# NYXFLOWER/TIP

Hardware: AMD Instinct MI355X
Metric: D-D edges aggregated/sec (encoder fwd+bwd) (higher is better)
Workload: dtype f32

## Files before the change

### include/tipk.h

```cpp
#ifndef TIPK_H
#define TIPK_H

#include <stdint.h>

#ifdef __cplusplus
extern "C" {
#endif

#define TIPK_ABI_VERSION 24

#define TIPK_OK            0
#define TIPK_EINVAL      (-1)
#define TIPK_EUNSUPPORTED (-2)
#define TIPK_EHIP_BASE   (-1000)

typedef void* tipk_stream_t;

int         tipk_abi_version(void);
const char* tipk_strerror(int status);
const char* tipk_build_id(void);
int         tipk_set_option(const char* name, int value);
int         tipk_get_option(const char* name, int* value);
int         tipk_device_info(int device, int* n_cu, int* lds_bytes_per_cu, int* wavefront, char* arch, int arch_len);

int tipk_gather_sum(const float* table, int64_t ld_table, int64_t n_table ,
                    const int32_t* row_id, const float* edge_w ,
                    const int32_t* items, int64_t n_items,
                    float* out, int64_t ld_out,
                    float* partial ,
                    const float* row_scale ,
                    const float* bias , int relu,
                    int d, int group_slots , tipk_stream_t stream);
// ... 122 lines not shown

int tipk_rgcn_dest_products_supported(int64_t n_nodes, int64_t n_rel, int n_bases, int d_in);
int tipk_rgcn_dest_products(const float* x, int64_t ld_x, int d_in, const float* att, int64_t ld_att, int n_bases,
                            int64_t n_nodes, int64_t n_rel, const int32_t* node_desc, const uint32_t* edges,
                            float* t, int64_t t_sb, int64_t t_sv, tipk_stream_t stream);

int tipk_sum_slabs_xb(const float* slabs, int64_t n_slabs, int64_t slab_stride, int64_t n_rows, int d_in,
                      const float* row_scale , const float* addend , int relu, float* x,
                      const float* basis, const float* root, int n_bases, int d_out, float* xb, float* xroot,
                      tipk_stream_t stream);

int tipk_rgcn_row_products_supported(int64_t n_nodes, int64_t n_rel, int n_bases, int channels);
int64_t tipk_rgcn_row_products_slabs(int64_t n_nodes, int channels);
int tipk_rgcn_row_products(const float* table, int64_t ld_table, int64_t n_nodes, int channels, const float* att,
                           int64_t ld_att, int64_t n_rel, int n_bases, const int32_t* entries, const int32_t* desc,
                           const float* xb , int64_t ld_xb, float* t, float* datt_slabs ,
                           tipk_stream_t stream);

int tipk_rgcn_row_products_s_supported(int64_t n_nodes, int64_t n_rel, int n_bases, int channels);
int tipk_rgcn_row_products_s(const float* table, int64_t ld_table, int64_t n_nodes, int channels, const float* att,
                             int64_t ld_att, int64_t n_rel, int n_bases, const int32_t* entries, const int32_t* desc,
                             const float* xb , int64_t ld_xb, float* t, float* datt_slabs ,
                             tipk_stream_t stream);

int tipk_transpose(const float* in, int64_t rows, int64_t cols, float* out, tipk_stream_t stream);

int tipk_rows_affine(const float* in, int64_t ld_in,
                     const float* row_mul, const float* row_div,
                     const float* gate, int64_t ld_gate,
                     float* out, int64_t ld_out,
                     int64_t rows, int64_t cols, int accumulate, tipk_stream_t stream);

int tipk_gate_colsum_groups(int64_t rows, int64_t cols);
int tipk_gate_colsum(const float* in, int64_t ld_in, const float* gate, int64_t ld_gate,
                     float* out, int64_t ld_out, int64_t rows, int64_t cols, float* scratch,
                     tipk_stream_t stream);

int tipk_drug_mix_fwd(const float* xd, int64_t ld_xd, const float* d_norm, const float* mean, int64_t ld_mean,
                      const float* w, int p, int q, int64_t rows, int ne, int cat, float* out, int64_t ld_out,
                      tipk_stream_t stream);

int tipk_drug_mix_gather_supported(int p, int q);
int tipk_drug_mix_gather_fwd(const float* xd, int64_t ld_xd, const float* d_norm, const float* h, int64_t ld_h,
                             const int32_t* ptr, const int32_t* src, const float* scale, const int32_t* wg_desc,
                             const int32_t* order , int64_t n_wg,
                             const float* w, int p, int q, int64_t rows, int ne, int cat, float* out, int64_t ld_out,
// ... 197 lines not shown
```

### tip_amd/_lib.py

```python
import ctypes as C
import glob
import hashlib
import os
import subprocess

import torch

_HERE = os.path.dirname(os.path.abspath(__file__))
LIB_PATH = os.path.join(_HERE, 'libtipk.so')
CSRC = os.path.join(_HERE, 'csrc')

ABI_VERSION = 24


class TipkError(RuntimeError):
    pass


class GemmDesc(C.Structure):
    _fields_ = [('m', C.c_int64), ('n', C.c_int64), ('k', C.c_int64),
                ('batch', C.c_int64), ('kbatch', C.c_int64), ('ksplit', C.c_int64),
                ('a', C.c_void_p), ('a_sm', C.c_int64), ('a_sk', C.c_int64), ('a_sq', C.c_int64), ('a_sz', C.c_int64),
                ('b', C.c_void_p), ('b_sk', C.c_int64), ('b_sn', C.c_int64), ('b_sq', C.c_int64), ('b_sz', C.c_int64),
                ('c', C.c_void_p), ('c_sm', C.c_int64), ('c_sz', C.c_int64), ('c_ss', C.c_int64),
                ('c_in', C.c_void_p), ('cin_sm', C.c_int64), ('cin_sz', C.c_int64),
                ('alpha', C.c_float), ('relu', C.c_int)]


class SlabSumDesc(C.Structure):
    _fields_ = [('in_', C.c_void_p), ('n_slabs', C.c_int64), ('slab_stride', C.c_int64), ('count', C.c_int64),
                ('alpha', C.c_float), ('accumulate', C.c_int),
                ('row_scale', C.c_void_p), ('cols', C.c_int64),
                ('addend', C.c_void_p), ('relu', C.c_int),
                ('gate', C.c_void_p),
                ('out', C.c_void_p)]
# ... 39 lines not shown
    'tipk_gather_sum': (_I, [_P, _L, _L, _P, _P, _P, _L, _P, _L, _P, _P, _P, _I, _I, _I, _P]),
    'tipk_gather_sum_finalize': (_I, [_P, _P, _L, _P, _L, _P, _P, _I, _I, _I, _P]),
    'tipk_gather_sum_riders_supported': (_I, [_I, _I]),
    'tipk_gather_sum_riders': (_I, [_P, _L, _L, _P, _P, _P, _L, _P, _L, _P, _P, _I, _I, _I, _P, _L, _P, C.POINTER(SlabSumDesc), C.c_int32, _P]),
    'tipk_gather_sum_lin_supported': (_I, [_I, _I, _I]),
    'tipk_gather_sum_lin': (_I, [_P, _L, _L, _P, _P, _P, _L, _P, _L, _P, _P, _L, _L, _P, _I, _P, _L, _I, _I, _I, _P]),
    'tipk_gather_rows_csr': (_I, [_P, _L, _L, _P, _P, _L, _P, _L, _I, _P]),
    'tipk_rel_gather_supported': (_I, [_L, _I, _I]),
    'tipk_rel_gather_occupancy': (_I, [_L, _I, _I]),
    'tipk_rel_gather_chunk': (_I, [_L, _I, _I]),
    'tipk_pair_product_supported': (_I, [_I, _I]),
    'tipk_pair_product': (_I, [_P, _P, _L, _L, _I, _I, _I, _I, _P, _P, _P, _P, _P]),
    'tipk_rgcn_pair_grads_supported': (_I, [_I, _I]),
    'tipk_rgcn_pair_grads': (_I, [_P, _L, _P, _P, _L, _L, _I, _I, _P, _P, _P, _L, _P, _L, _L, _P, _L, _P]),
    'tipk_stream_gather_parts': (_I, [_P, _L, _I, _L, _P, _L, _P, _L, _P, _P, _P, _I, _P, _P, _P, _L, _P]),
    'tipk_stream_gather_parts_two': (_I, [_P, _P, _L, _I, _L, _P, _L, _P, _L, _P, _P, _P, _I, _P, _P, _P, _P, _L, _P]),
    'tipk_rgcn_dest_products_supported': (_I, [_L, _L, _I, _I]),
    'tipk_rgcn_dest_products': (_I, [_P, _L, _I, _P, _L, _I, _L, _L, _P, _P, _P, _L, _L, _P]),
    'tipk_rgcn_row_products_supported': (_I, [_L, _L, _I, _I]),
    'tipk_rgcn_row_products_slabs': (_L, [_L, _I]),
    'tipk_rgcn_row_products': (_I, [_P, _L, _L, _I, _P, _L, _L, _I, _P, _P, _P, _L, _P, _P, _P]),
    'tipk_rgcn_row_products_s_supported': (_I, [_L, _L, _I, _I]),
    'tipk_rgcn_row_products_s': (_I, [_P, _L, _L, _I, _P, _L, _L, _I, _P, _P, _P, _L, _P, _P, _P]),
    'tipk_sum_slabs_xb': (_I, [_P, _L, _L, _L, _I, _P, _P, _I, _P, _P, _P, _I, _I, _P, _P, _P]),
    'tipk_stream_gather_supported': (_I, [_L, _I, _I]),
    'tipk_stream_gather_piece': (_I, []),
    'tipk_stream_gather_two': (_I, [_P, _P, _L, _L, _I, _L, _P, _P, _P, _I, _P, _P, _L, _P]),
    'tipk_stream_gather': (_I, [_P, _L, _L, _I, _L, _P, _P, _P, _I, _P, _P, _P, _P, _L, _I, _I, _P, _P, _I, _P]),
    'tipk_rel_gather': (_I, [_I, _P, _L, _L, _I, _L, _P, _P, _P, _I, _P, _P, _P, _P, _L, _P]),
    'tipk_gemm_f32': (_I, [C.POINTER(GemmDesc), _P]),
    'tipk_gemm_f32_group': (_I, [C.POINTER(GemmDesc), C.c_int32, _P]),
    'tipk_sum_slabs_group': (_I, [C.POINTER(SlabSumDesc), C.c_int32, _P]),
    'tipk_gemm_wg_group_supported': (_I, [C.POINTER(WgGemmDesc)]),
    'tipk_gemm_wg_group': (_I, [C.POINTER(WgGemmDesc), C.c_int32, C.POINTER(SlabSumDesc), C.c_int32, _P]),
    'tipk_rgcn_dy_products_plan': (_I, [_L, _L, _I, C.POINTER(_I), C.POINTER(_I)]),
    'tipk_rgcn_dy_products': (_I, [_P, _L, _P, _L, _P, _L, _L, _L, _I, _P, _L, _P, _P, _P]),
    'tipk_rgcn_node_products_plan': (_I, [_L, _I, _L, _I, C.POINTER(_I)]),
    'tipk_rgcn_node_products': (_I, [_P, _L, _I, _P, _P, _P, _L, _L, _P, _L, _I, _P, _L, _L, _P, _P, _L, _L, _P, _P]),
    'tipk_sum_slabs': (_I, [_P, _L, _L, _L, _F, _I, _P, _P]),
    'tipk_sum_slabs_ex': (_I, [_P, _L, _L, _L, _F, _I, _P, _L, _P, _I, _P, _P]),
    'tipk_transpose': (_I, [_P, _L, _L, _P, _P]),
    'tipk_rows_affine': (_I, [_P, _L, _P, _P, _P, _L, _P, _L, _L, _L, _I, _P]),
    'tipk_gate_colsum_groups': (_I, [_L, _L]),
    'tipk_gate_colsum': (_I, [_P, _L, _P, _L, _P, _L, _L, _L, _P, _P]),
    'tipk_drug_mix_fwd': (_I, [_P, _L, _P, _P, _L, _P, _I, _I, _L, _I, _I, _P, _L, _P]),
    'tipk_drug_mix_gather_supported': (_I, [_I, _I]),
# ... 177 lines not shown
```

### tip_amd/csrc/tipk_row_products.hip

```cpp
#include <stdlib.h>
#include <type_traits>
#include "tipk_common.h"

namespace {

typedef float f32x16 __attribute__((ext_vector_type(16)));
typedef unsigned int u32;
typedef __attribute__((address_space(3))) float rp_lds_f32_t;

constexpr int RP_WAVES = 8;
constexpr int RP_TLD = 33;

struct RpArgs {
    const float* table; u32 ld_table_b; int n_nodes, ch;
    const float* att; u32 ld_att_b; int R, NB;
    const float* xb; int64_t ld_xb;
    const int32_t* entries; const int32_t* desc; int n_tiles;
    float* t_out;
    float* datt;
    int n_groups;
    int dbg;
};

__device__ __forceinline__ float rp_ldg(const float* base, u32 byte_off) {
    return *reinterpret_cast<const float*>(reinterpret_cast<const char*>(base) + byte_off);
}
__device__ __forceinline__ float rp_and(float v, u32 mask) { return __uint_as_float(__float_as_uint(v) & mask); }
template <int I>
__device__ __forceinline__ u32 rp_row_bcast(u32 x) {
    return (u32)__builtin_amdgcn_update_dpp(0, (int)x, 0x150 + (I & 15), 0xf, 0xf, true);
}
template <int I>
__device__ __forceinline__ void rp_fmac_row_bcast(float& d, float x, float y) {
    asm("v_fmac_f32_dpp %0, %1, %2 row_newbcast:%3 row_mask:0xf bank_mask:0xf bound_ctrl:1" : "+v"(d) : "v"(x), "v"(y), "n"(I & 15));
}
__device__ __forceinline__ void rp_wave_sync() {
    __builtin_amdgcn_fence(__ATOMIC_RELEASE, "wavefront");
    __builtin_amdgcn_wave_barrier();
    __builtin_amdgcn_fence(__ATOMIC_ACQUIRE, "wavefront");
}
template <int N, int I = 0, typename F>
__device__ __forceinline__ void rp_static_for(F&& f) {
    if constexpr (I < N) {
// ... 191 lines not shown
                if constexpr ((g & 1) == 0) { consume(lo, va, wa); issue(lo_nx, va, g + 2 < NQ ? wa : wb); }
                else { consume(lo, vb, wa); issue(lo_nx, vb, g + 2 < NQ ? wa : wb); }
            });
            wa = wb; wb = wq[0];
#pragma unroll
            for (int q = 0; q + 1 < WQ; ++q) wq[q] = wq[q + 1];
            wq[WQ - 1] = load_word(b + 2 + WQ);
            ++b;
        } while (++i < nbat);
        finish_tile();
        nbat = nbat_next;
    }
    if (wave_on) {
#pragma unroll
        for (int q = 0; q < CPL; ++q)
#pragma unroll
            for (int r = 0; r < 16; ++r) {
                const int bb = (r & 3) + 8 * (r >> 2) + 4 * kh;
                if (bb < NB) a.t_out[(int64_t)bb * NC + col0 + 32 * q + row] = acc1[q][r];
            }
    }
}

constexpr int RPS_TS = 65;
constexpr int RPS_TILE = (33 * RPS_TS + 3) / 4 * 4;

template <bool P2>
__global__ __launch_bounds__(RP_WAVES * 64, 4) void row_products_s_kernel(RpArgs a) {
    constexpr int TS = RPS_TS;
    extern __shared__ __attribute__((aligned(16))) float lds[];
    const int t = threadIdx.x, lane = t & 63;
    const int w = __builtin_amdgcn_readfirstlane(t >> 6);
    const int row = lane & 31, kh = lane >> 5;
    float* tile = lds + w * RPS_TILE;
    float* attl = lds + RP_WAVES * RPS_TILE;
    const int cb = (int)blockIdx.x / a.n_groups, grp = (int)blockIdx.x - cb * a.n_groups;
    const int node_raw = grp * RP_WAVES + w;
    const bool wave_on = node_raw < a.n_nodes;
    const int node = wave_on ? node_raw : a.n_nodes - 1;
    const int NB = a.NB, R = a.R;
    const int64_t NC = (int64_t)a.n_nodes * a.ch;
    const int64_t col0 = (int64_t)node * a.ch + cb * 64;
    const u32 voff = (u32)(cb * 64 + lane) * 4u;
    u32 tile_base = __builtin_amdgcn_readfirstlane((u32)(uintptr_t)(rp_lds_f32_t*)tile);
    const u32 att_b = (u32)(row < NB ? row : NB - 1) * 4u;
    const __amdgpu_buffer_rsrc_t rsrc = __builtin_amdgcn_make_buffer_rsrc(const_cast<float*>(a.table), 0,
                                                                           (int)((u32)a.n_nodes * a.ld_table_b), 0x00020000);
    float xbv[2][16];
    if (P2) {
        const int64_t b_off = (int64_t)(row < NB ? row : NB - 1) * a.ld_xb + col0;
#pragma unroll
        for (int q = 0; q < 2; ++q)
#pragma unroll
            for (int kk = 0; kk < 16; ++kk)
                xbv[q][kk] = rp_and(a.xb[b_off + 32 * q + 2 * kk + kh], (row < NB && wave_on) ? 0xffffffffu : 0u);
    }
    f32x16 acc1[2];
#pragma unroll
    for (int q = 0; q < 2; ++q)
#pragma unroll
        for (int i = 0; i < 16; ++i) acc1[q][i] = 0.f;
    const int32_t* dsc = a.desc + (int64_t)node * a.n_tiles * 2;
    int b = __builtin_amdgcn_readfirstlane(dsc[0]);
    int nbat = __builtin_amdgcn_readfirstlane(dsc[1]);
    int tl = 0;
    float acc = 0.f;
    float atv[16];
    float va[8], vb[8];
    int w1c[16], wn[32];
    typedef const __attribute__((address_space(4))) int32_t* rp_const_i32_t;
    const rp_const_i32_t entries_c = (rp_const_i32_t)(uintptr_t)a.entries;
    auto load_words = [&](int batch, int (&dst)[32]) __attribute__((always_inline)) {
        const rp_const_i32_t eb = entries_c + (int64_t)batch * 32;
#pragma unroll
        for (int j = 0; j < 32; ++j) dst[j] = eb[j];
    };
    auto issue = [&](auto lo_c, float (&val)[8], const int (&w0)[32]) __attribute__((always_inline)) {
        constexpr int LO = decltype(lo_c)::value;
#pragma unroll
        for (int j = 0; j < 8; ++j)
            val[j] = __builtin_bit_cast(float, __builtin_amdgcn_raw_buffer_load_b32(rsrc, (int)voff, w0[LO + j], 0));
    };
    auto consume = [&](auto lo_c, float (&val)[8], const int (&w1)[16]) __attribute__((always_inline)) {
        constexpr int LO = decltype(lo_c)::value;
        const u32 tb = tile_base;
#pragma unroll
        for (int j = 0; j < 8; ++j) {
            const int wd = w1[LO + j];
            const float keep = __int_as_float(wd & 0x3f800000);
            acc = fmaf(acc, keep, val[j]);
            if (!TIPK_DBG(a.dbg & 2))
                asm volatile("s_add_u32 m0, %1, %2\n\ts_nop 0\n\tds_write_addtid_b32 %0" : : "v"(acc), "s"(tb), "s"(wd) : "memory", "scc");
        }
    };
    constexpr int NT = RP_WAVES * 64, PER = 1024 / NT;
    float att_next[PER];
    auto att_elem = [&](int tile_i, int i) __attribute__((always_inline)) {
        const int e = i * NT + t, r = tile_i * 32 + (e >> 5), bb = e & 31;
        const float v = a.att[(int64_t)(r < R ? r : R - 1) * (a.ld_att_b >> 2) + (bb < NB ? bb : NB - 1)];
        return rp_and(v, (r < R && bb < NB && tile_i < a.n_tiles) ? 0xffffffffu : 0u);
    };
    auto att_store = [&](int buf) __attribute__((always_inline)) {
#pragma unroll
        for (int i = 0; i < PER; ++i) attl[buf * (32 * RP_TLD) + ((i * NT + t) >> 5) * RP_TLD + (t & 31)] = att_next[i];
    };
    if (P2) {
#pragma unroll
        for (int i = 0; i < PER; ++i) att_next[i] = att_elem(0, i);
        att_store(0);
        __syncthreads();
    }
    auto begin_tile = [&]() __attribute__((always_inline)) {
        const int r0 = tl * 32;
        if (P2) {
#pragma unroll
            for (int i = 0; i < PER; ++i) att_next[i] = att_elem(tl + 1 < a.n_tiles ? tl + 1 : tl, i);
        } else {
            const float* att_t = a.att + (int64_t)r0 * (a.ld_att_b >> 2);
#pragma unroll
            for (int kk = 0; kk < 16; ++kk) {
                const int r = r0 + 2 * kk + kh;
                atv[kk] = rp_ldg(att_t, (u32)((r < R ? r : R - 1) - r0) * a.ld_att_b + att_b);
            }
            if (r0 + 32 > R || NB < 32) {
#pragma unroll
                for (int kk = 0; kk < 16; ++kk)
                    atv[kk] = rp_and(atv[kk], (r0 + 2 * kk + kh < R && row < NB) ? 0xffffffffu : 0u);
            }
        }
        constexpr int N4 = 32 * TS / 4;
        static_assert(32 * TS % 4 == 0, "tile zeroing");
#pragma unroll
        for (int i = 0; i < (N4 + 63) / 64; ++i)
            if (i * 64 + lane < N4) tipk_st4(tile + (i * 64 + lane) * 4, make_float4(0.f, 0.f, 0.f, 0.f));
        rp_wave_sync();
    };
    auto finish_tile = [&]() __attribute__((always_inline)) {
        const int r0 = tl * 32;
        rp_wave_sync();
        if (!TIPK_DBG(a.dbg & 4))
#pragma unroll
        for (int kk = 0; kk < 16; ++kk) {
            const float av = P2 ? attl[(tl & 1) * (32 * RP_TLD) + (2 * kk + kh) * RP_TLD + row] : atv[kk];
#pragma unroll
            for (int q = 0; q < 2; ++q)
                acc1[q] = __builtin_amdgcn_mfma_f32_32x32x2f32(av, tile[(2 * kk + kh) * TS + 32 * q + row], acc1[q], 0, 0, 0);
        }
        if (P2) {
            f32x16 acc2;
#pragma unroll
            for (int i = 0; i < 16; ++i) acc2[i] = 0.f;
#pragma unroll
            for (int q = 0; q < 2; ++q)
#pragma unroll
                for (int kk = 0; kk < 16; ++kk)
                    acc2 = __builtin_amdgcn_mfma_f32_32x32x2f32(tile[row * TS + 32 * q + 2 * kk + kh], xbv[q][kk], acc2, 0, 0, 0);
            att_store((tl + 1) & 1);
            rp_wave_sync();
#pragma unroll
            for (int r = 0; r < 16; ++r) {
                const int rr = (r & 3) + 8 * (r >> 2) + 4 * kh;
                tile[rr * 32 + row] = acc2[r];
            }
            __syncthreads();
#pragma unroll
            for (int i = 0; i < PER; ++i) {
                const int e = i * NT + t;
                float sum = lds[e];
#pragma unroll
                for (int q = 1; q < RP_WAVES; ++q) sum += lds[q * RPS_TILE + e];
                const int rr = r0 + (e >> 5), bb = e & 31;
                if (rr < R && bb < NB) a.datt[((int64_t)blockIdx.x * R + rr) * NB + bb] = sum;
            }
            __syncthreads();
        }
    };
    constexpr std::integral_constant<int, 0> c0{};
    constexpr std::integral_constant<int, 8> c8{};
    load_words(b, wn);
#pragma unroll
    for (int j = 0; j < 16; ++j) w1c[j] = wn[16 + j];
    issue(c0, va, wn);
    issue(c8, vb, wn);
    for (tl = 0; tl < a.n_tiles; ++tl) {
        const int nbat_next = __builtin_amdgcn_readfirstlane(dsc[2 * (tl + 1 < a.n_tiles ? tl + 1 : tl) + 1]);
        begin_tile();
        int i = 0;
        do {
            load_words(b + 1, wn);
            consume(c0, va, w1c);
            issue(c0, va, wn);
            consume(c8, vb, w1c);
            issue(c8, vb, wn);
#pragma unroll
            for (int j = 0; j < 16; ++j) w1c[j] = wn[16 + j];
            ++b;
        } while (++i < nbat);
        finish_tile();
        nbat = nbat_next;
    }
    if (wave_on) {
#pragma unroll
        for (int q = 0; q < 2; ++q)
#pragma unroll
            for (int r = 0; r < 16; ++r) {
                const int bb = (r & 3) + 8 * (r >> 2) + 4 * kh;
                if (bb < NB) a.t_out[(int64_t)bb * NC + col0 + 32 * q + row] = acc1[q][r];
            }
    }
}

template <bool P2>
int rps_launch(const RpArgs& a, unsigned blocks, hipStream_t st) {
    const size_t lds = (size_t)(RP_WAVES * RPS_TILE + (P2 ? 2 * 32 * RP_TLD : 0)) * sizeof(float);
    hipError_t e = hipFuncSetAttribute((const void*)row_products_s_kernel<P2>, hipFuncAttributeMaxDynamicSharedMemorySize, (int)lds);
    if (e != hipSuccess) return tipk_hip_status(e);
    hipLaunchKernelGGL((row_products_s_kernel<P2>), dim3(blocks), dim3(RP_WAVES * 64), lds, st, a);
    TIPK_RETURN_LAUNCH();
}

template <int CPL> constexpr size_t rp_lds_bytes(bool p2) {
    return (size_t)(RP_WAVES * RpGeom<CPL>::TILE + (p2 ? 2 * 32 * RP_TLD : 0)) * sizeof(float);
}

template <bool P2, int CPL>
int rp_launch(const RpArgs& a, unsigned blocks, hipStream_t st) {
    const size_t lds = rp_lds_bytes<CPL>(P2);
    hipError_t e = hipFuncSetAttribute((const void*)row_products_kernel<P2, CPL>, hipFuncAttributeMaxDynamicSharedMemorySize, (int)lds);
    if (e != hipSuccess) return tipk_hip_status(e);
    hipLaunchKernelGGL((row_products_kernel<P2, CPL>), dim3(blocks), dim3(RP_WAVES * 64), lds, st, a);
    TIPK_RETURN_LAUNCH();
}

inline int rp_cpl(int channels) { return channels % 64 == 0 ? 2 : 1; }

}

extern "C" int tipk_rgcn_row_products_supported(int64_t n_nodes, int64_t n_rel, int n_bases, int channels) {
    if (n_nodes <= 0 || n_rel <= 0 || n_bases <= 0 || n_bases > 32 || channels <= 0 || channels % 32 != 0) return 0;
    if (n_nodes > 65536 || n_rel > 0x7fffffffLL) return 0;
// ... 32 lines not shown

extern "C" int tipk_rgcn_row_products_s_supported(int64_t n_nodes, int64_t n_rel, int n_bases, int channels) {
    if (n_nodes <= 0 || n_rel <= 0 || n_bases <= 0 || n_bases > 32 || channels <= 0 || channels % 64 != 0) return 0;
    if (n_rel > 0x7fffffffLL || tipk_ceil_div(n_nodes, RP_WAVES) * (channels / 64) > 0x7fffffffLL) return 0;
    return 1;
}

extern "C" int tipk_rgcn_row_products_s(const float* table, int64_t ld_table, int64_t n_nodes, int channels, const float* att,
                                        int64_t ld_att, int64_t n_rel, int n_bases, const int32_t* entries, const int32_t* desc,
                                        const float* xb, int64_t ld_xb, float* t_out, float* datt_slabs, tipk_stream_t stream) {
    if (!tipk_rgcn_row_products_s_supported(n_nodes, n_rel, n_bases, channels)) return TIPK_EUNSUPPORTED;
    if (!table || !att || !entries || !desc || !t_out || ld_table < channels || ld_att < n_bases) return TIPK_EINVAL;
    if ((xb == nullptr) != (datt_slabs == nullptr) || (xb && ld_xb < n_nodes * channels)) return TIPK_EINVAL;
    if (n_nodes * ld_table * 4 >= (1LL << 31) || 32 * ld_att * 4 >= (1LL << 31)) return TIPK_EUNSUPPORTED;
    RpArgs a;
    a.table = table; a.ld_table_b = (u32)(ld_table * 4); a.n_nodes = (int)n_nodes; a.ch = channels;
    a.att = att; a.ld_att_b = (u32)(ld_att * 4); a.R = (int)n_rel; a.NB = n_bases;
    a.xb = xb; a.ld_xb = ld_xb;
    a.entries = entries; a.desc = desc; a.n_tiles = (int)tipk_ceil_div(n_rel, 32);
    a.t_out = t_out; a.datt = datt_slabs;
    a.n_groups = (int)tipk_ceil_div(n_nodes, RP_WAVES);
    a.dbg = TIPK_DBG(tipk_option(TIPK_OPT_DP_DEBUG));
    const unsigned blocks = (unsigned)(a.n_groups * (channels / 64));
    return xb ? rps_launch<true>(a, blocks, (hipStream_t)stream) : rps_launch<false>(a, blocks, (hipStream_t)stream);
}
```

### tip_amd/layers.py

```python
import math
import os
import pickle

import numpy as np
import torch
from torch import nn
from torch.nn import Parameter as Param

from . import encoder, ops, switches
from .data import Data, build_data_dict
from .neg_sampling import typed_negative_sampling
from .plan import (build_pair_bwd_plan, build_dest_plan, build_row_stream_plan, build_row_stream_plan_s, build_gather_plan, build_gather_plan_segmented, build_rel_plan, build_stream_plan, build_stream_plan_rows, build_csr_plan, group_slots_for,
                   relations_per_segment, DEFAULT_CHUNK)
from .utils import process_edges, auprc_auroc_ap_by_range

EPS = 1e-13

__all__ = ['GCNConv', 'MyRGCNConv', 'MyRGCNConv2', 'MyHierarchyConv', 'PPEncoder', 'FMEncoder',
           'FMEncoderCat', 'MultiInnerProductDecoder', 'NNDecoder', 'Setting', 'TIP']


def _ident(*tensors):
    key = []
    for t in tensors:
        if t is None:
            key.append(None)
        elif t.is_sparse:
            key.append((id(t), tuple(t.shape), str(t.device), t.dtype))
        else:
            key.append((t.data_ptr(), tuple(t.shape), t._version, str(t.device), t.dtype))
    return tuple(key)


class _PlanCache(object):

# ... 346 lines not shown
            pair_fwd = build_stream_plan_rows(src[keep] * n_nodes + dst[keep], rel[keep], n_nodes * n_nodes, n_rel, pair_wgs,
                                              (n_bases // split_p) // 4, ops.rel_stream_piece())
            pair_fwd.symmetric = symmetric
            pair_fwd.links = pair_link_words(src, dst, n_nodes)
        split_s = ops.rel_stream_split(n_nodes, d_out) if on_dev and n_rel * n_nodes < 2 ** 24 else 0
        if pair_fwd is not None and ops.pair_grads_supported(n_bases, d_out):
            sym, lanes_p = pair_fwd.symmetric, (n_bases // split_p) // 4
            pair_bwd = lambda: _shared_pair_bwd_plan(src, dst, rel, n_nodes, n_rel, 1.0 / deg, sym, pair_wgs, lanes_p, plan_share)
        if split_s:
            compact = bool(n_bases) and ops.node_products_slabs(n_nodes, d_out, n_rel, n_bases) > 0
            lanes_s = (d_out // split_s) // 4
            build_rs = lambda: build_stream_plan(src, dst, rel, n_nodes, n_rel, n_cu, lanes_s, ops.rel_stream_piece(), compact=compact)
            rs_bwd = build_rs if pair_bwd is not None else build_rs()
        else:
            rl_bwd = lambda: build_rel_plan(src, dst, rel, n_nodes, n_rel, wg_b, backward=True, lanes=lanes_b)
    dest_fwd = row_fwd = row_bwd = None
    wide = False
    if src.is_cuda and d_out and n_bases and pair_fwd is None and n_rel * n_nodes * d_out * 4 > (192 << 20):
        bits = ops.dest_products_bits(n_nodes, n_rel, n_bases, 1)
        if bits:
            dest_fwd = lambda: build_dest_plan(src, dst, rel, n_nodes, n_rel, bits)
        wide = bool(d_out) and d_out % 64 == 0 and ops.row_products_s_supported(n_nodes, n_rel, n_bases, d_out) \
            and n_nodes < (1 << 23) and n_nodes * d_out * 4 < 2 ** 31
        if wide:
            row_fwd = lambda: build_row_stream_plan_s(dst, src, rel, n_nodes, n_rel)
            row_bwd = lambda: build_row_stream_plan_s(src, dst, rel, n_nodes, n_rel)
        elif ops.row_products_supported(n_nodes, n_rel, n_bases, 32):
            row_fwd = lambda: build_row_stream_plan(dst, src, rel, n_nodes, n_rel)
            row_bwd = lambda: build_row_stream_plan(src, dst, rel, n_nodes, n_rel)

    def fwd_plan():
        y_bytes = n_rel * n_nodes * (d_out or 0) * 4
        ordered = rel.numel() < 2 or bool((rel[1:] >= rel[:-1]).all())
        if y_bytes > (192 << 20) and ordered:
            per = relations_per_segment(n_nodes, d_out)
            return build_gather_plan_segmented(dst, yrow, rel // per, n_nodes, n_rel * n_nodes, chunk, 'dd.fwd')
        return build_gather_plan(dst, yrow, n_nodes, n_rel * n_nodes, None, chunk, 'dd.fwd')

    return ops.AggGraph(fwd_plan,
                        lambda: build_gather_plan(yrow, dst, n_rel * n_nodes, n_nodes, None, chunk, 'dd.bwd'),
                        (1.0 / deg).contiguous(), rl_fwd, rl_bwd,
                        csr_bwd=lambda: build_csr_plan(yrow, dst, n_rel * n_nodes, n_nodes, 'dd.bwd'), rs_bwd=rs_bwd,
                        pair_fwd=pair_fwd, pair_bwd=pair_bwd, dest_fwd=dest_fwd, row_fwd=row_fwd, row_bwd=row_bwd,
                        row_wave_uniform=wide)


class _RGCNBase(nn.Module):
    def __init__(self, in_channels, out_channels, num_relations, num_bases, after_relu, bias=False,
# ... 408 lines not shown
```

### tip_amd/ops.py

```python
import os

import torch

from . import _lib, switches
from ._lib import SlabSumDesc, GemmDesc, WgGemmDesc, check, lib, ptr, stream_ptr, require_device

def _f32c(t):
    if t.dtype != torch.float32:
        raise _lib.TipkError('tip_amd computes in fp32; got %s' % t.dtype)
    if t.dim() >= 1 and t.stride(-1) != 1 and t.shape[-1] != 1:
        t = t.contiguous()
    return t


_TIMING = None


def timing_start():
    global _TIMING
    _TIMING = {}


def timing_stop():
    global _TIMING
# ... 426 lines not shown
    if switches.on('TIPK_NO_ROW_PRODUCTS'):
        return False
    return bool(lib().tipk_rgcn_row_products_supported(int(n_nodes), int(n_rel), int(nb), int(channels)))


def row_products_s_supported(n_nodes, n_rel, nb, channels):
    if switches.on('TIPK_NO_ROW_PRODUCTS_S'):
        return False
    return bool(lib().tipk_rgcn_row_products_s_supported(int(n_nodes), int(n_rel), int(nb), int(channels)))


def _row_plan(graph, transposed, n, r, nb, channels):
    if not graph.has_row_plans:
        return None
    if graph.row_plans_wave_uniform:
        if channels % 64 != 0 or not row_products_s_supported(n, r, nb, channels) or n * channels * 4 >= 2 ** 31:
            return None
    elif not row_products_supported(n, r, nb, channels):
        return None
    return graph.row_bwd if transposed else graph.row_fwd


def row_products(rp, table, att, xb2=None):
    if getattr(rp, 'ROW_BYTES', None) is not None:
        return _row_products_s(rp, table, att, xb2)
    return _row_products_v(rp, table, att, xb2)


def _row_products_s(rp, table, att, xb2=None):
    table, att = _f32c(table), _f32c(att)
    require_device(table, att, rp.entries)
    n, ch = table.shape
    r, nb = att.shape
    assert rp.n_nodes == n and rp.n_rel == r and table.stride(1) == 1 and att.stride(1) == 1
    entries = rp.entries_for(table.stride(0) * 4)
    t = torch.empty((nb, n, ch), dtype=torch.float32, device=table.device)
    slabs = None
    if xb2 is not None:
        assert xb2.shape == (nb, n * ch) and xb2.stride(1) == 1
        slabs = torch.empty((-(-n // 8) * (ch // 64), r, nb), dtype=torch.float32, device=table.device)
    with _timed('row_products_s[%dx%dx%d,edges=%d,%s]' % (n, nb, ch, rp.n_edges, 'T+datt' if slabs is not None else 'T')):
        check(lib().tipk_rgcn_row_products_s(ptr(table), table.stride(0), n, ch, ptr(att), att.stride(0), r, nb, ptr(entries),
                                             ptr(rp.desc), ptr(xb2), xb2.stride(0) if xb2 is not None else 0, ptr(t), ptr(slabs),
                                             stream_ptr(table.device)), 'tipk_rgcn_row_products_s')
    if slabs is None:
        return t
    return slab_job(slabs), t


def _row_products_v(rp, table, att, xb2=None):
    table, att = _f32c(table), _f32c(att)
    require_device(table, att, rp.entries)
    n, ch = table.shape
    r, nb = att.shape
    assert rp.n_nodes == n and rp.n_rel == r and table.stride(1) == 1 and att.stride(1) == 1
    if table.stride(0) % 64 != 0:
        wide = torch.empty((n, -(-ch // 64) * 64), dtype=torch.float32, device=table.device)
        wide[:, :ch] = table
        table = wide[:, :ch]
    t = torch.empty((nb, n, ch), dtype=torch.float32, device=table.device)
    slabs = None
    if xb2 is not None:
        assert xb2.shape == (nb, n * ch) and xb2.stride(1) == 1
        slabs = torch.empty((int(lib().tipk_rgcn_row_products_slabs(n, ch)), r, nb), dtype=torch.float32, device=table.device)
    with _timed('row_products[%dx%dx%d,edges=%d,%s]' % (n, nb, ch, rp.n_edges, 'T+datt' if slabs is not None else 'T')):
        check(lib().tipk_rgcn_row_products(ptr(table), table.stride(0), n, ch, ptr(att), att.stride(0), r, nb, ptr(rp.entries),
                                           ptr(rp.desc), ptr(xb2), xb2.stride(0) if xb2 is not None else 0, ptr(t), ptr(slabs),
# ... 1419 lines not shown
```

### tip_amd/plan.py

```python

import torch

DEFAULT_CHUNK = None
TARGET_ITEMS = 65536


def auto_chunk(n_edges):
    target = TARGET_ITEMS * 2 if n_edges <= (1 << 22) else TARGET_ITEMS
    c = 16
    while c < 128 and n_edges // c > target:
        c *= 2
    return c


ITEM_DIRECT, ITEM_PIECE, ITEM_LEADER, ITEM_NULL = 1, 2, 4, 8


class GatherPlan(object):

    def __init__(self, n_out, n_table, row_id, edge_w, items, split_rows, n_slots, perm, chunk, tag='',
                 group_slots=0):
        self.tag = tag
        self.n_out, self.n_table = int(n_out), int(n_table)
        self.row_id, self.edge_w = row_id, edge_w
# ... 993 lines not shown
    n_seg = n_nodes * n_tiles
    seg = key * n_tiles + rel // 32
    row_key = key * n_rel + rel
    order = torch.sort(row_key, stable=True).indices
    seg_s, row_s = seg[order], row_key[order]
    n_in = torch.bincount(seg_s, minlength=n_seg)
    nbat = torch.clamp((n_in + 15) // 16, min=1)
    first = torch.cumsum(nbat, 0) - nbat
    n_batches = int(nbat.sum())
    entries = torch.zeros((n_batches + 8, 2, 16), dtype=torch.int32, device=dev)
    entries[:, 1, :] = 32 * RowStreamPlanS.ROW_BYTES
    if e:
        seg_first = torch.cumsum(n_in, 0) - n_in
        pos = torch.arange(e, device=dev) - seg_first[seg_s]
        inside = torch.zeros(e, dtype=torch.int64, device=dev)
        inside[1:] = (row_s[1:] == row_s[:-1]).to(torch.int64)
        flat0 = (first[seg_s] + pos // 16) * 32 + pos % 16
        entries.view(-1)[flat0] = other[order].to(torch.int32)
        entries.view(-1)[flat0 + 16] = ((rel[order] % 32) * RowStreamPlanS.ROW_BYTES + inside * 0x3f800000).to(torch.int32)
    desc = torch.stack([first, nbat], dim=1).to(torch.int32).view(n_nodes, n_tiles, 2).contiguous()
    return RowStreamPlanS(n_nodes, n_rel, entries.contiguous(), desc, e)


def execute_row_stream_s_reference(plan, table, att, xb=None):
    n, r, nt = plan.n_nodes, plan.n_rel, plan.n_tiles
    table, att = table.double().cpu(), att.double().cpu()
    ent = plan.entries.cpu().to(torch.int64)
    desc = plan.desc.cpu().to(torch.int64)
    ch = table.shape[1]
    s = torch.zeros((nt * 32 + 1, n, ch), dtype=torch.float64)
    for v in range(n):
        for tl in range(nt):
            f, nb_ = int(desc[v, tl, 0]), int(desc[v, tl, 1])
            oth = ent[f:f + nb_, 0, :].reshape(-1)
            w1 = ent[f:f + nb_, 1, :].reshape(-1)
            row = (w1 & 0xffff) // RowStreamPlanS.ROW_BYTES
            rows = torch.where(row < 32, tl * 32 + row, torch.full_like(row, nt * 32))
            s[:, v].index_add_(0, rows, table[oth])
    s = s[:r]
    t = torch.einsum('rb,rvc->bvc', att, s)
    if xb is None:
        return t
    return t, torch.einsum('rvc,bvc->rb', s, xb.double().cpu())


def execute_row_stream_reference(plan, table, att, xb=None):
# ... 23 lines not shown
```

### tip_amd/switches.py

```python
import os

SWITCHES = {
    'TIPK_NO_ENCODER_STEP': 'FMEncoder.forward on the per-layer autograd nodes instead of tip_amd/encoder.py',
    'TIPK_NO_RELLOCAL': 'no LDS-resident D-D kernels (rel_gather / stream_gather): the generic gather route',
    'TIPK_NO_DY_FUSED': 'the two products of dY as two grouped GEMMs instead of tipk_rgcn_dy_products',
    'TIPK_NO_CELLS_TWO': 'the pair cells of the two R-GCN layers in two launches',
    'TIPK_NO_DEST_FWD': 'large graphs: the forward pass through Y instead of tipk_rgcn_dest_products',
    'TIPK_NO_ROW_PRODUCTS': 'large graphs: no tipk_rgcn_row_products',
    'TIPK_NO_ROW_PRODUCTS_S': 'large graphs: no tipk_rgcn_row_products_s (wave-uniform form)',
    'TIPK_NO_LAYER_HANDOVER': 'the slab sum between the R-GCN layers as a launch of its own',
    'TIPK_NO_PAIR_BWD': 'the round-4 backward route (compact dY + node_products) behind a pair-form forward pass',
    'TIPK_NO_SYMMETRIC_POS': 'the fused objective evaluates every directed positive (no weight-2 halves)',
    'TIPK_FLOAT_ATOMICS': 'the fused objective on float atomics (not bitwise reproducible)',
    'TIPK_NO_BITMAP': 'the sampler on the binary-search kernel instead of the LDS bitmap',
    'TIPK_NO_PAIR_PRODUCT': 'the pair product on the tiled GEMM instead of tipk_pair_product',
}
_forced = {}


def on(name):
    assert name in SWITCHES, name
    if name in _forced:
        return bool(_forced[name])
    return bool(os.environ.get(name))


def set(name, value):
    assert name in SWITCHES, name
    if value is None:
        _forced.pop(name, None)
    else:
        _forced[name] = bool(value)
# ... 1 lines not shown
```

Before: 39.78 billion.

## Pack occupied relation rows per tile in row-products kernel to skip empty MFMAs

Adds a packed-row variant of the wave-uniform row-products kernel. For each (node, relation-tile) the plan compacts only the relation rows that actually have edges, stores their count (nnz) and a byte-packed row map. The kernel then skips MFMA steps for empty rows and avoids zeroing the whole LDS tile, and it scatters the dAtt results back through the row map. A 16x16x4 MFMA variant with optional relation relabeling is also added. This is intended to cut wasted matrix work and LDS traffic on sparse relation tiles, at the cost of extra plan metadata loads and indirection, and a wider tile stride.

```diff
diff --git a/include/tipk.h b/include/tipk.h
--- a/include/tipk.h
+++ b/include/tipk.h
@@ -7,7 +7,7 @@
 extern "C" {
 #endif
 
-#define TIPK_ABI_VERSION 24
+#define TIPK_ABI_VERSION 25
 
 #define TIPK_OK            0
 #define TIPK_EINVAL      (-1)
@@ -176,6 +176,11 @@
                              int64_t ld_att, int64_t n_rel, int n_bases, const int32_t* entries, const int32_t* desc,
                              const float* xb , int64_t ld_xb, float* t, float* datt_slabs ,
                              tipk_stream_t stream);
+
+int tipk_rgcn_row_products_sp(const float* table, int64_t ld_table, int64_t n_nodes, int channels, const float* att,
+                              int64_t ld_att, int64_t n_rel, int n_bases, const int32_t* entries, const int32_t* desc,
+                              const int32_t* rows, const int32_t* rel_of , const float* xb ,
+                              int64_t ld_xb, float* t, float* datt_slabs , tipk_stream_t stream);
 
 int tipk_transpose(const float* in, int64_t rows, int64_t cols, float* out, tipk_stream_t stream);
 
diff --git a/tip_amd/_lib.py b/tip_amd/_lib.py
--- a/tip_amd/_lib.py
+++ b/tip_amd/_lib.py
@@ -10,7 +10,7 @@
 LIB_PATH = os.path.join(_HERE, 'libtipk.so')
 CSRC = os.path.join(_HERE, 'csrc')
 
-ABI_VERSION = 24
+ABI_VERSION = 25
 
 
 class TipkError(RuntimeError):
@@ -96,6 +96,7 @@
     'tipk_rgcn_row_products': (_I, [_P, _L, _L, _I, _P, _L, _L, _I, _P, _P, _P, _L, _P, _P, _P]),
     'tipk_rgcn_row_products_s_supported': (_I, [_L, _L, _I, _I]),
     'tipk_rgcn_row_products_s': (_I, [_P, _L, _L, _I, _P, _L, _L, _I, _P, _P, _P, _L, _P, _P, _P]),
+    'tipk_rgcn_row_products_sp': (_I, [_P, _L, _L, _I, _P, _L, _L, _I, _P, _P, _P, _P, _P, _L, _P, _P, _P]),
     'tipk_sum_slabs_xb': (_I, [_P, _L, _L, _L, _I, _P, _P, _I, _P, _P, _P, _I, _I, _P, _P, _P]),
     'tipk_stream_gather_supported': (_I, [_L, _I, _I]),
     'tipk_stream_gather_piece': (_I, []),
diff --git a/tip_amd/csrc/tipk_row_products.hip b/tip_amd/csrc/tipk_row_products.hip
--- a/tip_amd/csrc/tipk_row_products.hip
+++ b/tip_amd/csrc/tipk_row_products.hip
@@ -19,6 +19,8 @@
     float* t_out;
     float* datt;
     int n_groups;
+    const int32_t* rows;
+    const int32_t* rel_of;
     int dbg;
 };
 
@@ -256,12 +258,15 @@
     }
 }
 
-constexpr int RPS_TS = 65;
-constexpr int RPS_TILE = (33 * RPS_TS + 3) / 4 * 4;
-
-template <bool P2>
+template <bool PK> struct RpsGeom {
+    static constexpr int TS = PK ? 66 : 65;
+    static constexpr int TILE = (33 * TS + 3) / 4 * 4;
+    static constexpr int DS = PK ? 4 : 2;
+};
+
+template <bool P2, bool PK, bool HALVES>
 __global__ __launch_bounds__(RP_WAVES * 64, 4) void row_products_s_kernel(RpArgs a) {
-    constexpr int TS = RPS_TS;
+    constexpr int TS = RpsGeom<PK>::TS, RPS_TILE = RpsGeom<PK>::TILE, DS = RpsGeom<PK>::DS;
     extern __shared__ __attribute__((aligned(16))) float lds[];
     const int t = threadIdx.x, lane = t & 63;
     const int w = __builtin_amdgcn_readfirstlane(t >> 6);
@@ -281,7 +286,17 @@
     const __amdgpu_buffer_rsrc_t rsrc = __builtin_amdgcn_make_buffer_rsrc(const_cast<float*>(a.table), 0,
                                                                            (int)((u32)a.n_nodes * a.ld_table_b), 0x00020000);
     float xbv[2][16];
-    if (P2) {
+    if (P2 && HALVES) {
+        const int bq = lane & 15, kq = lane >> 4;
+#pragma unroll
+        for (int g = 0; g < 2; ++g) {
+            const int bb = 16 * g + bq;
+            const int64_t b_off = (int64_t)(bb < NB ? bb : NB - 1) * a.ld_xb + col0;
+#pragma unroll
+            for (int kk = 0; kk < 16; ++kk)
+                xbv[g][kk] = rp_and(a.xb[b_off + 4 * kk + kq], (bb < NB && wave_on) ? 0xffffffffu : 0u);
+        }
+    } else if (P2) {
         const int64_t b_off = (int64_t)(row < NB ? row : NB - 1) * a.ld_xb + col0;
 #pragma unroll
         for (int q = 0; q < 2; ++q)
@@ -294,10 +309,12 @@
     for (int q = 0; q < 2; ++q)
 #pragma unroll
         for (int i = 0; i < 16; ++i) acc1[q][i] = 0.f;
-    const int32_t* dsc = a.desc + (int64_t)node * a.n_tiles * 2;
+    const int32_t* dsc = a.desc + (int64_t)node * a.n_tiles * DS;
     int b = __builtin_amdgcn_readfirstlane(dsc[0]);
     int nbat = __builtin_amdgcn_readfirstlane(dsc[1]);
     int tl = 0;
+    int nnz = 32;
+    int pw[8];
     float acc = 0.f;
     float atv[16];
     float va[8], vb[8];
@@ -329,10 +346,17 @@
     };
     constexpr int NT = RP_WAVES * 64, PER = 1024 / NT;
     float att_next[PER];
+    auto rel_at = [&](int r) __attribute__((always_inline)) {
+        if (PK && a.rel_of) return r < a.n_tiles * 32 ? a.rel_of[r] : -1;
+        return r < R ? r : -1;
+    };
     auto att_elem = [&](int tile_i, int i) __attribute__((always_inline)) {
-        const int e = i * NT + t, r = tile_i * 32 + (e >> 5), bb = e & 31;
-        const float v = a.att[(int64_t)(r < R ? r : R - 1) * (a.ld_att_b >> 2) + (bb < NB ? bb : NB - 1)];
-        return rp_and(v, (r < R && bb < NB && tile_i < a.n_tiles) ? 0xffffffffu : 0u);
+        const int e = i * NT + t, r = rel_at(tile_i * 32 + (e >> 5)), bb = e & 31;
+        const float v = a.att[(int64_t)(r >= 0 ? r : 0) * (a.ld_att_b >> 2) + (bb < NB ? bb : NB - 1)];
+        return rp_and(v, (r >= 0 && bb < NB && tile_i < a.n_tiles) ? 0xffffffffu : 0u);
+    };
+    auto prow = [&](int kk) __attribute__((always_inline)) {
+        return ((u32)pw[kk >> 1] >> (16 * (kk & 1) + 8 * kh)) & 0xffu;
     };
     auto att_store = [&](int buf) __attribute__((always_inline)) {
 #pragma unroll
@@ -344,11 +368,30 @@
         att_store(0);
         __syncthreads();
     }
+    auto load_rows = [&]() __attribute__((always_inline)) {
+        const rp_const_i32_t rw = (rp_const_i32_t)(uintptr_t)a.rows + ((int64_t)node * a.n_tiles + tl) * 8;
+#pragma unroll
+        for (int j = 0; j < 8; ++j) pw[j] = rw[j];
+    };
     auto begin_tile = [&]() __attribute__((always_inline)) {
         const int r0 = tl * 32;
+        if (PK) nnz = __builtin_amdgcn_readfirstlane(dsc[DS * tl + 2]);
+        if (PK && !P2) load_rows();
         if (P2) {
 #pragma unroll
             for (int i = 0; i < PER; ++i) att_next[i] = att_elem(tl + 1 < a.n_tiles ? tl + 1 : tl, i);
+        } else if (PK && a.rel_of) {
+#pragma unroll
+            for (int kk = 0; kk < 16; ++kk) {
+                const int r = a.rel_of[r0 + (int)prow(kk)];
+                atv[kk] = rp_and(rp_ldg(a.att, (u32)(r >= 0 ? r : 0) * a.ld_att_b + att_b), (r >= 0 && row < NB) ? 0xffffffffu : 0u);
+            }
+        } else if (PK) {
+#pragma unroll
+            for (int kk = 0; kk < 16; ++kk) {
+                const int r = r0 + (int)prow(kk);
+                atv[kk] = rp_and(rp_ldg(a.att, (u32)(r < R ? r : 0) * a.ld_att_b + att_b), (r < R && row < NB) ? 0xffffffffu : 0u);
+            }
         } else {
             const float* att_t = a.att + (int64_t)r0 * (a.ld_att_b >> 2);
 #pragma unroll
@@ -362,25 +405,78 @@
                     atv[kk] = rp_and(atv[kk], (r0 + 2 * kk + kh < R && row < NB) ? 0xffffffffu : 0u);
             }
         }
-        constexpr int N4 = 32 * TS / 4;
-        static_assert(32 * TS % 4 == 0, "tile zeroing");
-#pragma unroll
-        for (int i = 0; i < (N4 + 63) / 64; ++i)
-            if (i * 64 + lane < N4) tipk_st4(tile + (i * 64 + lane) * 4, make_float4(0.f, 0.f, 0.f, 0.f));
+        if (PK && !P2) {
+            if (nnz & 1) tile[nnz * TS + lane] = 0.f;
+        } else {
+            constexpr int N4 = 32 * TS / 4;
+            static_assert(32 * TS % 4 == 0, "tile zeroing");
+#pragma unroll
+            for (int i = 0; i < (N4 + 63) / 64; ++i)
+                if (i * 64 + lane < N4) tipk_st4(tile + (i * 64 + lane) * 4, make_float4(0.f, 0.f, 0.f, 0.f));
+        }
         rp_wave_sync();
     };
     auto finish_tile = [&]() __attribute__((always_inline)) {
         const int r0 = tl * 32;
+        if (PK && P2) load_rows();
         rp_wave_sync();
         if (!TIPK_DBG(a.dbg & 4))
 #pragma unroll
         for (int kk = 0; kk < 16; ++kk) {
-            const float av = P2 ? attl[(tl & 1) * (32 * RP_TLD) + (2 * kk + kh) * RP_TLD + row] : atv[kk];
+            if (PK && 2 * kk >= nnz) break;
+            if (PK) asm volatile("");
+            const int ar = PK ? (int)prow(kk) : 2 * kk + kh;
+            const float av = P2 ? attl[(tl & 1) * (32 * RP_TLD) + ar * RP_TLD + row] : atv[kk];
 #pragma unroll
             for (int q = 0; q < 2; ++q)
                 acc1[q] = __builtin_amdgcn_mfma_f32_32x32x2f32(av, tile[(2 * kk + kh) * TS + 32 * q + row], acc1[q], 0, 0, 0);
         }
-        if (P2) {
+        if (P2 && HALVES) {
+            typedef float f32x4 __attribute__((ext_vector_type(4)));
+            f32x4 acc2[2][2];
+#pragma unroll
+            for (int h = 0; h < 2; ++h)
+#pragma unroll
+                for (int g = 0; g < 2; ++g)
+#pragma unroll
+                    for (int i = 0; i < 4; ++i) acc2[h][g][i] = 0.f;
+            if (!TIPK_DBG(a.dbg & 4))
+#pragma unroll
+            for (int h = 0; h < 2; ++h) {
+                if (16 * h >= nnz) break;
+                asm volatile("");
+#pragma unroll
+                for (int kk = 0; kk < 16; ++kk) {
+                    const float sv = tile[(16 * h + (lane & 15)) * TS + 4 * kk + (lane >> 4)];
+#pragma unroll
+                    for (int g = 0; g < 2; ++g) acc2[h][g] = __builtin_amdgcn_mfma_f32_16x16x4f32(sv, xbv[g][kk], acc2[h][g], 0, 0, 0);
+                }
+            }
+            att_store((tl + 1) & 1);
+            rp_wave_sync();
+            const int q4 = lane >> 4;
+#pragma unroll
+            for (int h = 0; h < 2; ++h) {
+                const u32 wsel = q4 == 0 ? (u32)pw[4 * h] : q4 == 1 ? (u32)pw[4 * h + 1] : q4 == 2 ? (u32)pw[4 * h + 2] : (u32)pw[4 * h + 3];
+#pragma unroll
+                for (int i = 0; i < 4; ++i) {
+                    const u32 tr = (wsel >> (8 * i)) & 0xffu;
+#pragma unroll
+                    for (int g = 0; g < 2; ++g) tile[tr * 32 + 16 * g + (lane & 15)] = acc2[h][g][i];
+                }
+            }
+            __syncthreads();
+#pragma unroll
+            for (int i = 0; i < PER; ++i) {
+                const int e = i * NT + t;
+                float sum = lds[e];
+#pragma unroll
+                for (int q = 1; q < RP_WAVES; ++q) sum += lds[q * RPS_TILE + e];
+                const int rr = rel_at(r0 + (e >> 5)), bb = e & 31;
+                if (rr >= 0 && bb < NB) a.datt[((int64_t)blockIdx.x * R + rr) * NB + bb] = sum;
+            }
+            __syncthreads();
+        } else if (P2) {
             f32x16 acc2;
 #pragma unroll
             for (int i = 0; i < 16; ++i) acc2[i] = 0.f;
@@ -394,7 +490,8 @@
 #pragma unroll
             for (int r = 0; r < 16; ++r) {
                 const int rr = (r & 3) + 8 * (r >> 2) + 4 * kh;
-                tile[rr * 32 + row] = acc2[r];
+                const u32 tr = PK ? ((u32)(kh ? pw[2 * (r >> 2) + 1] : pw[2 * (r >> 2)]) >> (8 * (r & 3))) & 0xffu : (u32)rr;
+                tile[tr * 32 + row] = acc2[r];
             }
             __syncthreads();
 #pragma unroll
@@ -403,8 +500,8 @@
                 float sum = lds[e];
 #pragma unroll
                 for (int q = 1; q < RP_WAVES; ++q) sum += lds[q * RPS_TILE + e];
-                const int rr = r0 + (e >> 5), bb = e & 31;
-                if (rr < R && bb < NB) a.datt[((int64_t)blockIdx.x * R + rr) * NB + bb] = sum;
+                const int rr = rel_at(r0 + (e >> 5)), bb = e & 31;
+                if (rr >= 0 && bb < NB) a.datt[((int64_t)blockIdx.x * R + rr) * NB + bb] = sum;
             }
             __syncthreads();
         }
@@ -417,7 +514,7 @@
     issue(c0, va, wn);
     issue(c8, vb, wn);
     for (tl = 0; tl < a.n_tiles; ++tl) {
-        const int nbat_next = __builtin_amdgcn_readfirstlane(dsc[2 * (tl + 1 < a.n_tiles ? tl + 1 : tl) + 1]);
+        const int nbat_next = __builtin_amdgcn_readfirstlane(dsc[DS * (tl + 1 < a.n_tiles ? tl + 1 : tl) + 1]);
         begin_tile();
         int i = 0;
         do {
@@ -444,12 +541,12 @@
     }
 }
 
-template <bool P2>
+template <bool P2, bool PK, bool HALVES = false>
 int rps_launch(const RpArgs& a, unsigned blocks, hipStream_t st) {
-    const size_t lds = (size_t)(RP_WAVES * RPS_TILE + (P2 ? 2 * 32 * RP_TLD : 0)) * sizeof(float);
-    hipError_t e = hipFuncSetAttribute((const void*)row_products_s_kernel<P2>, hipFuncAttributeMaxDynamicSharedMemorySize, (int)lds);
+    const size_t lds = (size_t)(RP_WAVES * RpsGeom<PK>::TILE + (P2 ? 2 * 32 * RP_TLD : 0)) * sizeof(float);
+    hipError_t e = hipFuncSetAttribute((const void*)row_products_s_kernel<P2, PK, HALVES>, hipFuncAttributeMaxDynamicSharedMemorySize, (int)lds);
     if (e != hipSuccess) return tipk_hip_status(e);
-    hipLaunchKernelGGL((row_products_s_kernel<P2>), dim3(blocks), dim3(RP_WAVES * 64), lds, st, a);
+    hipLaunchKernelGGL((row_products_s_kernel<P2, PK, HALVES>), dim3(blocks), dim3(RP_WAVES * 64), lds, st, a);
     TIPK_RETURN_LAUNCH();
 }
 
@@ -528,5 +625,28 @@
     a.n_groups = (int)tipk_ceil_div(n_nodes, RP_WAVES);
     a.dbg = TIPK_DBG(tipk_option(TIPK_OPT_DP_DEBUG));
     const unsigned blocks = (unsigned)(a.n_groups * (channels / 64));
-    return xb ? rps_launch<true>(a, blocks, (hipStream_t)stream) : rps_launch<false>(a, blocks, (hipStream_t)stream);
-}
+    a.rows = nullptr; a.rel_of = nullptr;
+    return xb ? rps_launch<true, false>(a, blocks, (hipStream_t)stream) : rps_launch<false, false>(a, blocks, (hipStream_t)stream);
+}
+
+extern "C" int tipk_rgcn_row_products_sp(const float* table, int64_t ld_table, int64_t n_nodes, int channels, const float* att,
+                                         int64_t ld_att, int64_t n_rel, int n_bases, const int32_t* entries, const int32_t* desc,
+                                         const int32_t* rows, const int32_t* rel_of, const float* xb, int64_t ld_xb, float* t_out,
+                                         float* datt_slabs, tipk_stream_t stream) {
+    if (!tipk_rgcn_row_products_s_supported(n_nodes, n_rel, n_bases, channels)) return TIPK_EUNSUPPORTED;
+    if (!table || !att || !entries || !desc || !rows || !t_out || ld_table < channels || ld_att < n_bases) return TIPK_EINVAL;
+    if ((xb == nullptr) != (datt_slabs == nullptr) || (xb && ld_xb < n_nodes * channels)) return TIPK_EINVAL;
+    if (n_nodes * ld_table * 4 >= (1LL << 31) || n_rel * ld_att * 4 >= (1LL << 31)) return TIPK_EUNSUPPORTED;
+    RpArgs a;
+    a.table = table; a.ld_table_b = (u32)(ld_table * 4); a.n_nodes = (int)n_nodes; a.ch = channels;
+    a.att = att; a.ld_att_b = (u32)(ld_att * 4); a.R = (int)n_rel; a.NB = n_bases;
+    a.xb = xb; a.ld_xb = ld_xb;
+    a.entries = entries; a.desc = desc; a.n_tiles = (int)tipk_ceil_div(n_rel, 32);
+    a.rows = rows; a.rel_of = rel_of;
+    a.t_out = t_out; a.datt = datt_slabs;
+    a.n_groups = (int)tipk_ceil_div(n_nodes, RP_WAVES);
+    a.dbg = TIPK_DBG(tipk_option(TIPK_OPT_DP_DEBUG));
+    const unsigned blocks = (unsigned)(a.n_groups * (channels / 64));
+    if (!xb) return rps_launch<false, true>(a, blocks, (hipStream_t)stream);
+    return rel_of ? rps_launch<true, true, true>(a, blocks, (hipStream_t)stream) : rps_launch<true, true, false>(a, blocks, (hipStream_t)stream);
+}
diff --git a/tip_amd/layers.py b/tip_amd/layers.py
--- a/tip_amd/layers.py
+++ b/tip_amd/layers.py
@@ -10,7 +10,7 @@
 from . import encoder, ops, switches
 from .data import Data, build_data_dict
 from .neg_sampling import typed_negative_sampling
-from .plan import (build_pair_bwd_plan, build_dest_plan, build_row_stream_plan, build_row_stream_plan_s, build_gather_plan, build_gather_plan_segmented, build_rel_plan, build_stream_plan, build_stream_plan_rows, build_csr_plan, group_slots_for,
+from .plan import (build_pair_bwd_plan, build_dest_plan, build_row_stream_plan, build_row_stream_plan_s, build_row_stream_plan_sp, build_gather_plan, build_gather_plan_segmented, build_rel_plan, build_stream_plan, build_stream_plan_rows, build_csr_plan, group_slots_for,
                    relations_per_segment, DEFAULT_CHUNK)
 from .utils import process_edges, auprc_auroc_ap_by_range
 
@@ -403,8 +403,11 @@
             dest_fwd = lambda: build_dest_plan(src, dst, rel, n_nodes, n_rel, bits)
         wide = bool(d_out) and d_out % 64 == 0 and ops.row_products_s_supported(n_nodes, n_rel, n_bases, d_out) \
             and n_nodes < (1 << 23) and n_nodes * d_out * 4 < 2 ** 31
-        if wide:
+        if wide and switches.on('TIPK_NO_ROW_PACKING'):
             row_fwd = lambda: build_row_stream_plan_s(dst, src, rel, n_nodes, n_rel)
+            row_bwd = lambda: build_row_stream_plan_s(src, dst, rel, n_nodes, n_rel)
+        elif wide:
+            row_fwd = lambda: build_row_stream_plan_sp(dst, src, rel, n_nodes, n_rel)
             row_bwd = lambda: build_row_stream_plan_s(src, dst, rel, n_nodes, n_rel)
         elif ops.row_products_supported(n_nodes, n_rel, n_bases, 32):
             row_fwd = lambda: build_row_stream_plan(dst, src, rel, n_nodes, n_rel)
diff --git a/tip_amd/ops.py b/tip_amd/ops.py
--- a/tip_amd/ops.py
+++ b/tip_amd/ops.py
@@ -472,12 +472,14 @@
 
 
 def row_products(rp, table, att, xb2=None):
+    if getattr(rp, 'rows', None) is not None:
+        return _row_products_s(rp, table, att, xb2, packed=True)
     if getattr(rp, 'ROW_BYTES', None) is not None:
         return _row_products_s(rp, table, att, xb2)
     return _row_products_v(rp, table, att, xb2)
 
 
-def _row_products_s(rp, table, att, xb2=None):
+def _row_products_s(rp, table, att, xb2=None, packed=False):
     table, att = _f32c(table), _f32c(att)
     require_device(table, att, rp.entries)
     n, ch = table.shape
@@ -489,10 +491,14 @@
     if xb2 is not None:
         assert xb2.shape == (nb, n * ch) and xb2.stride(1) == 1
         slabs = torch.empty((-(-n // 8) * (ch // 64), r, nb), dtype=torch.float32, device=table.device)
-    with _timed('row_products_s[%dx%dx%d,edges=%d,%s]' % (n, nb, ch, rp.n_edges, 'T+datt' if slabs is not None else 'T')):
-        check(lib().tipk_rgcn_row_products_s(ptr(table), table.stride(0), n, ch, ptr(att), att.stride(0), r, nb, ptr(entries),
-                                             ptr(rp.desc), ptr(xb2), xb2.stride(0) if xb2 is not None else 0, ptr(t), ptr(slabs),
-                                             stream_ptr(table.device)), 'tipk_rgcn_row_products_s')
+    name = 'tipk_rgcn_row_products_sp' if packed else 'tipk_rgcn_row_products_s'
+    plan_args = (ptr(rp.desc), ptr(rp.rows), ptr(rp.rel_of)) if packed else (ptr(rp.desc),)
+    if packed:
+        require_device(rp.desc, rp.rows, rp.rel_of)
+    with _timed('%s[%dx%dx%d,edges=%d,%s]' % (name[10:], n, nb, ch, rp.n_edges, 'T+datt' if slabs is not None else 'T')):
+        check(getattr(lib(), name)(ptr(table), table.stride(0), n, ch, ptr(att), att.stride(0), r, nb, ptr(entries), *plan_args,
+                                   ptr(xb2), xb2.stride(0) if xb2 is not None else 0, ptr(t), ptr(slabs),
+                                   stream_ptr(table.device)), name)
     if slabs is None:
         return t
     return slab_job(slabs), t
diff --git a/tip_amd/plan.py b/tip_amd/plan.py
--- a/tip_amd/plan.py
+++ b/tip_amd/plan.py
@@ -1039,6 +1039,98 @@
     return RowStreamPlanS(n_nodes, n_rel, entries.contiguous(), desc, e)
 
 
+class RowStreamPlanSP(RowStreamPlanS):
+    ROW_BYTES = 264
+
+    def __init__(self, n_nodes, n_rel, entries, desc, rows, rel_of, n_edges):
+        super().__init__(n_nodes, n_rel, entries, desc, n_edges)
+        self.rows, self.rel_of = rows, rel_of
+
+    def to(self, device):
+        return RowStreamPlanSP(self.n_nodes, self.n_rel, self.entries.to(device), self.desc.to(device), self.rows.to(device),
+                               None if self.rel_of is None else self.rel_of.to(device), self.n_edges)
+
+    def tile_rows(self):
+        w = self.rows.to(torch.int64).view(self.n_nodes, self.n_tiles, 8, 1)
+        return ((w >> (8 * torch.arange(4, device=w.device))) & 0xff).view(self.n_nodes, self.n_tiles, 32)
+
+
+def row_order_by_size(rel, n_rel):
+    sizes = torch.bincount(rel.to(torch.int64).cpu(), minlength=int(n_rel))
+    return torch.sort(-sizes, stable=True).indices
+
+
+def build_row_stream_plan_sp(key, other, rel, n_nodes, n_rel, order=None):
+    dev = key.device
+    n_nodes, n_rel = int(n_nodes), int(n_rel)
+    n_tiles = (n_rel + 31) // 32
+    key, other, rel = key.to(torch.int64), other.to(torch.int64), rel.to(torch.int64)
+    rel_of = None
+    if order is not None:
+        order = order.to(device=dev, dtype=torch.int64)
+        assert order.numel() == n_rel and bool((torch.sort(order).values == torch.arange(n_rel, device=dev)).all())
+        label = torch.empty(n_rel, dtype=torch.int64, device=dev)
+        label[order] = torch.arange(n_rel, device=dev)
+        rel = label[rel]
+        rel_of = torch.full((n_tiles * 32,), -1, dtype=torch.int32, device=dev)
+        rel_of[:n_rel] = order.to(torch.int32)
+    e = int(key.numel())
+    n_seg = n_nodes * n_tiles
+    seg = key * n_tiles + rel // 32
+    row_key = key * (n_tiles * 32) + rel
+    order_e = torch.sort(row_key, stable=True).indices
+    seg_s, row_s = seg[order_e], row_key[order_e]
+    n_in = torch.bincount(seg_s, minlength=n_seg)
+    nbat = torch.clamp((n_in + 15) // 16, min=1)
+    first = torch.cumsum(nbat, 0) - nbat
+    n_batches = int(nbat.sum())
+    occ = torch.zeros(n_seg * 32, dtype=torch.bool, device=dev)
+    occ[row_s] = True
+    occ = occ.view(n_seg, 32)
+    nnz = occ.sum(1)
+    local = torch.arange(32, device=dev).expand(n_seg, 32)
+    tile_rows = torch.sort(torch.where(occ, local, local + 32), dim=1).values % 32
+    packed = (torch.cumsum(occ.to(torch.int64), 1) - 1).view(-1)
+    rows = (tile_rows.view(n_seg, 8, 4) << (8 * torch.arange(4, device=dev))).sum(2).to(torch.int32)
+    entries = torch.zeros((n_batches + 8, 2, 16), dtype=torch.int32, device=dev)
+    entries[:, 1, :] = 32 * RowStreamPlanSP.ROW_BYTES
+    if e:
+        seg_first = torch.cumsum(n_in, 0) - n_in
+        pos = torch.arange(e, device=dev) - seg_first[seg_s]
+        inside = torch.zeros(e, dtype=torch.int64, device=dev)
+        inside[1:] = (row_s[1:] == row_s[:-1]).to(torch.int64)
+        flat0 = (first[seg_s] + pos // 16) * 32 + pos % 16
+        entries.view(-1)[flat0] = other[order_e].to(torch.int32)
+        entries.view(-1)[flat0 + 16] = (packed[row_s] * RowStreamPlanSP.ROW_BYTES + inside * 0x3f800000).to(torch.int32)
+    desc = torch.stack([first, nbat, nnz, torch.zeros_like(nnz)], dim=1).to(torch.int32).view(n_nodes, n_tiles, 4).contiguous()
+    return RowStreamPlanSP(n_nodes, n_rel, entries.contiguous(), desc, rows.view(n_nodes, n_tiles, 8).contiguous(), rel_of, e)
+
+
+def execute_row_stream_sp_reference(plan, table, att, xb=None):
+    n, r, nt = plan.n_nodes, plan.n_rel, plan.n_tiles
+    table, att = table.double().cpu(), att.double().cpu()
+    ent = plan.entries.cpu().to(torch.int64)
+    desc = plan.desc.cpu().to(torch.int64)
+    trow = plan.tile_rows().cpu()
+    rel_of = torch.arange(nt * 32) if plan.rel_of is None else plan.rel_of.cpu().to(torch.int64)
+    rel_of = torch.where((rel_of >= 0) & (rel_of < r), rel_of, torch.full_like(rel_of, r))
+    ch = table.shape[1]
+    s = torch.zeros((r + 1, n, ch), dtype=torch.float64)
+    for v in range(n):
+        for tl in range(nt):
+            f, nb_ = int(desc[v, tl, 0]), int(desc[v, tl, 1])
+            oth = ent[f:f + nb_, 0, :].reshape(-1)
+            p = (ent[f:f + nb_, 1, :].reshape(-1) & 0xffff) // RowStreamPlanSP.ROW_BYTES
+            keep = p < 32
+            rows = rel_of[tl * 32 + trow[v, tl][p[keep]]]
+            s[:, v].index_add_(0, rows, table[oth[keep]])
+    s = s[:r]
+    t = torch.einsum('rb,rvc->bvc', att, s)
+    if xb is None:
+        return t
+    return t, torch.einsum('rvc,bvc->rb', s, xb.double().cpu())
+
+
 def execute_row_stream_s_reference(plan, table, att, xb=None):
     n, r, nt = plan.n_nodes, plan.n_rel, plan.n_tiles
     table, att = table.double().cpu(), att.double().cpu()
diff --git a/tip_amd/switches.py b/tip_amd/switches.py
--- a/tip_amd/switches.py
+++ b/tip_amd/switches.py
@@ -8,6 +8,7 @@
     'TIPK_NO_DEST_FWD': 'large graphs: the forward pass through Y instead of tipk_rgcn_dest_products',
     'TIPK_NO_ROW_PRODUCTS': 'large graphs: no tipk_rgcn_row_products',
     'TIPK_NO_ROW_PRODUCTS_S': 'large graphs: no tipk_rgcn_row_products_s (wave-uniform form)',
+    'TIPK_NO_ROW_PACKING': 'large graphs: the wave-uniform row plans without packed rows (tipk_rgcn_row_products_s, not _sp)',
     'TIPK_NO_LAYER_HANDOVER': 'the slab sum between the R-GCN layers as a launch of its own',
     'TIPK_NO_PAIR_BWD': 'the round-4 backward route (compact dY + node_products) behind a pair-form forward pass',
     'TIPK_NO_SYMMETRIC_POS': 'the fused objective evaluates every directed positive (no weight-2 halves)',
```

New measurement: 39.54 billion (median of 6 runs). No clear change (-0.6%).
